# xiejihong0306/collision-detect-GJK-EPA

Measured on AMD Instinct MI355X. Metric: M convex-pair GJK+EPA queries/sec at 1/2/4/8 MI355X; % HBM roofline, higher is better.
Workload: dtype f64

## Files before the change

### collision-detect-gjk-epa_amd/csrc/gjkepa_kernel.h

```cpp
#pragma once
#include <hip/hip_runtime.h>

#include <cstddef>
#include <cstdint>

#ifndef GJKEPA_G0_G
#define GJKEPA_G0_G 4
#endif
#ifndef GJKEPA_G0_K
#define GJKEPA_G0_K 8
#endif
#ifndef GJKEPA_G0_MINW
#define GJKEPA_G0_MINW 2
#endif
#ifndef GJKEPA_G1_G
#define GJKEPA_G1_G 16
#endif
#ifndef GJKEPA_G1_K
#define GJKEPA_G1_K 8
#endif
#ifndef GJKEPA_G1_MINW
#define GJKEPA_G1_MINW 3
#endif
#ifndef GJKEPA_G2_G
// ... 50 lines not shown
#ifndef GJKEPA_E2_VCAP
#define GJKEPA_E2_VCAP 72
#endif
#ifndef GJKEPA_E2_FCAP
#define GJKEPA_E2_FCAP 128
#endif
#ifndef GJKEPA_E2_MINW
#define GJKEPA_E2_MINW 2
#endif
#ifndef GJKEPA_E2_REFILL
#define GJKEPA_E2_REFILL 1
#endif
#ifndef GJKEPA_E3_G
#define GJKEPA_E3_G 64
#endif
#ifndef GJKEPA_E3_K
#define GJKEPA_E3_K 4
#endif
#ifndef GJKEPA_E3_VCAP
#define GJKEPA_E3_VCAP 40
#endif
#ifndef GJKEPA_E3_FCAP
#define GJKEPA_E3_FCAP 64
#endif
#ifndef GJKEPA_E3_MINW
#define GJKEPA_E3_MINW 4
#endif
#ifndef GJKEPA_E4_G
#define GJKEPA_E4_G 64
#endif
#ifndef GJKEPA_E4_K
#define GJKEPA_E4_K 4
#endif
#ifndef GJKEPA_E4_VCAP
#define GJKEPA_E4_VCAP 104
#endif
#ifndef GJKEPA_E4_FCAP
#define GJKEPA_E4_FCAP 208
#endif
#ifndef GJKEPA_E4_MINW
#define GJKEPA_E4_MINW 2
#endif
#ifndef GJKEPA_E5_G
#define GJKEPA_E5_G 64
#endif
#ifndef GJKEPA_E5_K
#define GJKEPA_E5_K 4
#endif
#ifndef GJKEPA_E5_VCAP
#define GJKEPA_E5_VCAP 208
#endif
#ifndef GJKEPA_E5_FCAP
#define GJKEPA_E5_FCAP 416
#endif
#ifndef GJKEPA_E5_MINW
#define GJKEPA_E5_MINW 1
#endif
#ifndef GJKEPA_Q_VCAP
#define GJKEPA_Q_VCAP 40
#endif
#ifndef GJKEPA_Q_FCAP
#define GJKEPA_Q_FCAP 64
#endif
#ifndef GJKEPA_C0_G
#define GJKEPA_C0_G 8
#endif
#ifndef GJKEPA_C0_K
#define GJKEPA_C0_K 4
#endif
#ifndef GJKEPA_C0_MINW
#define GJKEPA_C0_MINW 3
#endif
#ifndef GJKEPA_C1_G
#define GJKEPA_C1_G 64
#endif
#ifndef GJKEPA_C1_K
#define GJKEPA_C1_K 4
#endif
#ifndef GJKEPA_C1_MINW
#define GJKEPA_C1_MINW 3
#endif
#ifndef GJKEPA_CT_QUEUE04
#define GJKEPA_CT_QUEUE04 1
#endif
#ifndef GJKEPA_SEED_HANDOFF
#define GJKEPA_SEED_HANDOFF 1
#endif
#ifndef GJKEPA_E1_PRIO
#define GJKEPA_E1_PRIO 2
#endif
#ifndef GJKEPA_SCREEN_MIN_K
#define GJKEPA_SCREEN_MIN_K 8
#endif
#ifndef GJKEPA_G0_LH
#define GJKEPA_G0_LH 1
#endif
#ifndef GJKEPA_G1_LH
#define GJKEPA_G1_LH 1
#endif
#ifndef GJKEPA_G2_LH
#define GJKEPA_G2_LH 1
#endif
#ifndef GJKEPA_E0_LH
#define GJKEPA_E0_LH 1
#endif
#ifndef GJKEPA_E1_LH
#define GJKEPA_E1_LH 0
#endif
#ifndef GJKEPA_E2_LH
#define GJKEPA_E2_LH 0
#endif
#ifndef GJKEPA_E3_LH
#define GJKEPA_E3_LH 1
#endif
#ifndef GJKEPA_E4_LH
#define GJKEPA_E4_LH 1
#endif
#ifndef GJKEPA_E5_LH
#define GJKEPA_E5_LH 0
#endif
#ifndef GJKEPA_C0_LH
#define GJKEPA_C0_LH 1
#endif
#ifndef GJKEPA_C1_LH
#define GJKEPA_C1_LH 1
#endif
#define GJKEPA_GJK_TIERS 3
#define GJKEPA_EPA_TIERS 6
#define GJKEPA_CONTACT_TIERS 2

#define GJKEPA_WS_COUNTERS 40
#define GJKEPA_WS_TALLY 48
#define GJKEPA_ROUTE_DONE 0
#define GJKEPA_ROUTE_GJK1 1
#define GJKEPA_ROUTE_EPA0 0x10
#define GJKEPA_ROUTE_CT0 0x20
#define GJKEPA_ROUTE_CT(t) (GJKEPA_ROUTE_CT0 + 2 * (t))
#define GJKEPA_ROUTE_REDO 0x2E
#define GJKEPA_TALLY_SEED_OWN 0x2D
#define GJKEPA_TALLY_SEED_HANDED 0x2F

#define GJKEPA_PARK_VC 72
#define GJKEPA_PARK_FC 128
#define GJKEPA_PARK_HDR 128
#define GJKEPA_PARK_BYTES (GJKEPA_PARK_HDR + 3 * 8 * GJKEPA_PARK_VC + 2 * 4 * GJKEPA_PARK_FC)

#define GJKEPA_GRID_UNITS (-2)

struct gjkepa_gjk_args {
    const void* verts;
    const int64_t* hull_off;
    const int32_t* hull_cnt;
    const int32_t* pairs;
    int64_t n_pairs;
    uint8_t* route;
    int route_code;
    uint32_t* ctr;
    int claim;
    uint32_t* tally;
    uint32_t* warm;
    void* out;
    int grid;
    int num_cus;
    uint32_t guard;
};

struct gjkepa_epa_args {
    int version;
    double tol_ff;
    const void* verts;
    const int64_t* hull_off;
    const int32_t* hull_cnt;
    const int32_t* pairs;
    int64_t n_pairs;
    uint8_t* route;
    int route_code;
    int next_code;
    int ct_base;
    uint32_t* ctr;
    int claim;
    uint32_t* tally;
    void* out;
    int grid;
    int num_cus;
    unsigned char* park;
    uint32_t* park_ctr;
    uint32_t park_cap;
    uint32_t guard;
};

__host__ __device__ inline uint64_t gjkepa_mix(uint64_t h, uint64_t v) {
    h ^= v + 0x9e3779b97f4a7c15ull + (h << 6) + (h >> 2);
    return h;
}
__host__ __device__ inline uint32_t gjkepa_fold(uint64_t h) { return (uint32_t)(h ^ (h >> 32)) | 1u; }
__host__ __device__ inline uint32_t gjkepa_guard_of(const gjkepa_gjk_args& a) {
    uint64_t h = 0x67ull;
    h = gjkepa_mix(h, (uint64_t)a.verts); h = gjkepa_mix(h, (uint64_t)a.hull_off); h = gjkepa_mix(h, (uint64_t)a.hull_cnt);
    h = gjkepa_mix(h, (uint64_t)a.pairs); h = gjkepa_mix(h, (uint64_t)a.n_pairs); h = gjkepa_mix(h, (uint64_t)a.route);
    h = gjkepa_mix(h, (uint64_t)(int64_t)a.route_code); h = gjkepa_mix(h, (uint64_t)a.ctr);
    h = gjkepa_mix(h, (uint64_t)(int64_t)a.claim); h = gjkepa_mix(h, (uint64_t)a.tally); h = gjkepa_mix(h, (uint64_t)a.warm);
    h = gjkepa_mix(h, (uint64_t)a.out); h = gjkepa_mix(h, (uint64_t)(int64_t)a.grid); h = gjkepa_mix(h, (uint64_t)(int64_t)a.num_cus);
    return gjkepa_fold(h);
}
__host__ __device__ inline uint32_t gjkepa_guard_of(const gjkepa_epa_args& a) {
    uint64_t h = 0x65ull;
    h = gjkepa_mix(h, (uint64_t)(int64_t)a.version); h = gjkepa_mix(h, __builtin_bit_cast(uint64_t, a.tol_ff));
    h = gjkepa_mix(h, (uint64_t)a.verts); h = gjkepa_mix(h, (uint64_t)a.hull_off); h = gjkepa_mix(h, (uint64_t)a.hull_cnt);
    h = gjkepa_mix(h, (uint64_t)a.pairs); h = gjkepa_mix(h, (uint64_t)a.n_pairs); h = gjkepa_mix(h, (uint64_t)a.route);
    h = gjkepa_mix(h, (uint64_t)(int64_t)a.route_code); h = gjkepa_mix(h, (uint64_t)(int64_t)a.next_code);
    h = gjkepa_mix(h, (uint64_t)(int64_t)a.ct_base); h = gjkepa_mix(h, (uint64_t)a.ctr);
    h = gjkepa_mix(h, (uint64_t)(int64_t)a.claim); h = gjkepa_mix(h, (uint64_t)a.tally); h = gjkepa_mix(h, (uint64_t)a.out);
    h = gjkepa_mix(h, (uint64_t)(int64_t)a.grid); h = gjkepa_mix(h, (uint64_t)(int64_t)a.num_cus);
    h = gjkepa_mix(h, (uint64_t)a.park); h = gjkepa_mix(h, (uint64_t)a.park_ctr); h = gjkepa_mix(h, (uint64_t)a.park_cap);
    return gjkepa_fold(h);
}

#ifndef GJKEPA_D0_MINW
#define GJKEPA_D0_MINW 2
#endif
#ifndef GJKEPA_D1_MINW
#define GJKEPA_D1_MINW 2
#endif
// ... 117 lines not shown
```

### collision-detect-gjk-epa_amd/csrc/gjkepa_kernel.hip

```cpp
#include <hip/hip_runtime.h>

#include <cfloat>
#include <cmath>
#include <cstdint>
#include <type_traits>

#include "../../include/gjkepa.h"
#include "gjkepa_kernel.h"
#include "gk_common.h"

#ifdef GK_PART
#define GK_IN(p) (GK_PART == (p))
#else
#define GK_IN(p) 1
#endif
#if GK_IN(12) || GK_IN(14)
#include "dist_simplex.h"
#endif
#if GK_IN(13)
#include "cast_advance.h"
#endif
#if GK_IN(14)
#include "manifold_clip.h"
#endif
// ... 1296 lines not shown
    const V3<T> q = vmk<T>(n.x, n.y, T(0));
    const T nq = norm2(q);
    nnew = vdiv(q, nq);
    return 0;
}

constexpr uint32_t kStale = 0xFFFFFFFFu;
constexpr int PH_MISS = 0, PH_HIT = -1;

CTX_T DEV V3<T> support_pt(const CTX& c, V3<T> d, uint32_t& code) {
    int ia, ib;
    support_idx(c, d, ia, ib);
    code = (uint32_t)ia | ((uint32_t)ib << 16);
    return vsub(c.A(ia), c.B(ib));
}
CTX_T DEV V3<T> decode_pt(const CTX& c, uint32_t code) {
    if (code == kStale) return zero3<T>();
    return vsub(c.A((int)(code & 0xffffu)), c.B((int)(code >> 16)));
}

CTX_T DEV void update_simplex_c(const CTX& c, V3<T> nq, V3<T>& s0, V3<T>& s1, V3<T>& s2, V3<T>& s3,
                                uint32_t& k0, uint32_t& k1, uint32_t& k2, uint32_t& k3) {
    const V3<T> M = centroid4(s0, s1, s2, s3), O = zero3<T>();
    const int q = c.g.gl & 3;
    const V3<T> ref = q == 3 ? s1 : s0;
    if (dot(nq, vsub(ref, M)) < T(0)) nq = vneg(nq);
    T best = dot(vneg(nq), vsub(ref, O));
    int k = q;
    V3<T> dir = nq;
#pragma unroll
    for (int st = 0; st < 2; ++st) {
        const T ob = st == 0 ? xchg<0>(best) : xchg<1>(best);
        const int ok = st == 0 ? xchg<0>(k) : xchg<1>(k);
        const V3<T> od = st == 0 ? vmk<T>(xchg<0>(dir.x), xchg<0>(dir.y), xchg<0>(dir.z))
                                 : vmk<T>(xchg<1>(dir.x), xchg<1>(dir.y), xchg<1>(dir.z));
        const bool take = ob > best || (ob == best && ok < k);
        best = take ? ob : best;
        k = take ? ok : k;
        dir = vsel(take, od, dir);
    }
    k = c.g.uni(k);
    uint32_t km;
    const V3<T> SM = support_pt(c, dir, km);
    const V3<T> o0 = s0, o1 = s1, o2 = s2;
    const uint32_t c0 = k0, c1 = k1, c2 = k2, c3 = k3;
    s0 = vsel(k == 3, o1, o0);
    s1 = vsel(k == 0 || k == 3, o2, o1);
    s2 = vsel(k == 2, o2, s3);
    s3 = SM;
    k0 = k == 3 ? c1 : c0;
    k1 = (k == 0 || k == 3) ? c2 : c1;
    k2 = k == 2 ? c2 : c3;
    k3 = km;
}

constexpr double kWarmMargin = 1e-6;
constexpr uint32_t kWarmMiss = 0xFFFFFFFEu;
CTX_T DEV bool warm_start(CTX& c, const uint32_t* w, uint32_t* kc) {
    uint32_t code[4];
    bool ok = true;
#pragma unroll
    for (int i = 0; i < 4; ++i) {
        code[i] = w[i];
        ok = ok && code[i] != kStale && (int)(code[i] & 0xffffu) < c.na && (int)(code[i] >> 16) < c.nb;
    }
    if (!c.g.unib(ok)) return false;
    const V3<T> s0 = decode_pt(c, code[0]), s1 = decode_pt(c, code[1]), s2 = decode_pt(c, code[2]), s3 = decode_pt(c, code[3]);
    const V3<T> M = centroid4(s0, s1, s2, s3), O = zero3<T>();
    const V3<T> P[4] = {s0, s1, s2, s3};
    const int F[4][3] = {{0, 2, 3}, {0, 1, 3}, {0, 1, 2}, {1, 2, 3}};
    bool inside = true;
#pragma unroll
    for (int f = 0; f < 4; ++f) {
        V3<T> n = face_nml(P[F[f][0]], P[F[f][1]], P[F[f][2]]);
        if (dot(n, vsub(P[F[f][0]], M)) < T(0)) n = vneg(n);
        inside = inside && dot(vsub(P[F[f][0]], O), n) > T(kWarmMargin);
    }
    if (!c.g.unib(inside)) return false;
#pragma unroll
    for (int i = 0; i < 4; ++i) kc[i] = code[i];
    return true;
}

CTX_T DEV int gjk_phase(CTX& c, uint32_t* kc, int& gjk_it, SeedOut<T>* so = nullptr) {
    const V3<T> O = zero3<T>();
    auto& L = c.L;
    const int gl = c.g.gl;
    gjk_it = 0;
    {
        T cs[(6 + G - 1) / G];
#pragma unroll
        for (int j0 = 0; j0 < 6; j0 += G) {
            const int j = j0 + gl;
            cs[j0 / G] = T(0);
            if (j < 6) {
                const int h = j / 3, ax = j - 3 * (j / 3);
                const TH* col = ax == 0 ? L.hx[h] : ax == 1 ? L.hy[h] : L.hz[h];
                const int n = h ? c.nb : c.na;
                T sum = 0;
                int i = 0;
                for (; i + 8 <= n; i += 8) {
                    TH v[8];
#pragma unroll
                    for (int u = 0; u < 8; ++u) v[u] = col[i + u];
#pragma unroll
                    for (int u = 0; u < 8; ++u) sum += (T)v[u];
                }
                for (; i < n; ++i) sum += (T)col[i];
                cs[j0 / G] = sum / (T)n;
            }
        }
        const int gb = c.g.lane & ~(G - 1);
        auto mc = [&](int j) { return __shfl(cs[j / G], gb + j % G); };
        const V3<T> m1 = vmk<T>(mc(0), mc(1), mc(2)), m2 = vmk<T>(mc(3), mc(4), mc(5));
        T r1 = -Tol<T>::BIG, r2 = -Tol<T>::BIG;
#pragma unroll
        for (int k = 0; k < K; ++k) {
            int i = k * G + gl;
            const V3<T> da = vsub(c.AV(k), m1);
            const T ta = da.x * da.x + da.y * da.y + da.z * da.z;
            if (i < c.na && ta > r1) r1 = ta;
            const V3<T> db = vsub(c.BV(k), m2);
            const T tb = db.x * db.x + db.y * db.y + db.z * db.z;
            if (i < c.nb && tb > r2) r2 = tb;
        }
        r1 = tsqrt(gmax<G>(r1));
        r2 = tsqrt(gmax<G>(r2));
        GK_STAMP(SG_SPHERE);
        if (!c.g.unib(norm2(vsub(m1, m2)) <= r1 + r2 + T(1))) return PH_MISS;
    }
    V3<T> s0 = O, s1 = O, s2 = O, s3 = O;
    uint32_t k0 = kStale, k1 = kStale, k2 = kStale, k3 = kStale;
    V3<T> dir;
    for (int iter = 1;; ++iter) {
        if (iter > 99) return PH_MISS;
        dir = vmk<T>((T)kDirTab[iter - 1][0], (T)kDirTab[iter - 1][1], (T)kDirTab[iter - 1][2]);
        s0 = support_pt(c, dir, k0);
        dir = vneg(dir);
        s1 = support_pt(c, dir, k1);
        if (!c.g.unib(allclose8(s0, s1))) break;
    }
    dir = vec_pl(O, s0, s1);
    s2 = support_pt(c, dir, k2);
    if (c.g.unib(allclose8(s2, s0) || allclose8(s2, s1))) return PH_MISS;
    dir = utzvec(cross(vsub(s1, s0), vsub(s2, s1)));
    const T vd = dot(vsub(O, s2), dir);
    bool enter = false;
    if (c.g.unib(fabs(vd) < Tol<T>::PT) && c.g.unib(inside_tri(s0, s1, s2, O))) enter = true;
    const bool tri = enter;
    const int q = gl & 3;
    V3<T> nq = zero3<T>();
    T mdq = 0;
    if (!enter) {
        if (c.g.unib(vd < T(0))) dir = vneg(dir);
        s3 = support_pt(c, dir, k3);
        const V3<T> n = uninml(s0, s1, s2);
        if (c.g.unib(is_zero_nml(n))) return GJKEPA_STATUS_DEGENERATE;
        if (c.g.unib(fabs(dot(vsub(s3, s0), n)) < Tol<T>::PT)) return PH_MISS;
        nq = quad_normal(q, s0, s1, s2, s3, mdq);
        if (c.g.unib(quad_inside(q, s0, s1, s2, s3, nq))) enter = true;
    }
    GK_STAMP(SG_INIT);
    if (!enter) {
        constexpr int HS = (12 + G - 1) / G;
        T h1[HS], h2[HS];
#pragma unroll
        for (int t = 0; t < HS; ++t) { h1[t] = 0; h2[t] = 0; }
        const uint64_t lowg = G == 64 ? ~0ull : ((1ull << (G & 63)) - 1ull);
        const int sh = c.g.lane & ~(G - 1);
        for (int it = 1;; ++it) {
            gjk_it = it;
            if (it > 50) return PH_MISS;
#pragma unroll
            for (int t = 0; t < HS; ++t) {
                const int j = t * G + gl;
                h2[t] = h1[t];
                h1[t] = simplex_coord(j < 12 ? j : 0, s0, s1, s2, s3);
            }
            GK_STAMP(SG_CHK);
            update_simplex_c(c, nq, s0, s1, s2, s3, k0, k1, k2, k3);
            nq = quad_normal(q, s0, s1, s2, s3, mdq);
            GK_STAMP(SG_UPD);
            if (c.g.unib(qbcast<2>(mdq) < Tol<T>::PT)) return PH_MISS;
            const V3<T> n = vmk<T>(qbcast<2>(nq.x), qbcast<2>(nq.y), qbcast<2>(nq.z));
            if (c.g.unib(fabs(dot(vsub(s3, s0), n)) < Tol<T>::PT)) return PH_MISS;
            if (c.g.unib(quad_inside(q, s0, s1, s2, s3, nq))) break;
            uint32_t e1 = 0, e2 = 0;
#pragma unroll
            for (int t = 0; t < HS; ++t) {
                const int j = t * G + gl;
                const T cur = simplex_coord(j < 12 ? j : 0, s0, s1, s2, s3);
                e1 |= (uint32_t)((__ballot(fabs(cur - h1[t]) < Tol<T>::PT) >> sh) & lowg) << (t * G);
                e2 |= (uint32_t)((__ballot(fabs(cur - h2[t]) < Tol<T>::PT) >> sh) & lowg) << (t * G);
            }
            e1 &= 0xFFFu;
            e2 &= 0xFFFu;
            bool over = true;
#pragma unroll
            for (int p = 0; p < 4; ++p) over = over && (((e1 >> (3 * p)) & 7u) == 7u || ((e2 >> (3 * p)) & 7u) == 7u);
            if (c.g.unib(over)) return PH_MISS;
        }
        GK_STAMP(SG_CHK);
    }
    kc[0] = k0; kc[1] = k1; kc[2] = k2; kc[3] = k3;
    if constexpr (handoff<T>()) {
        if (so) {
            const bool same_bits = c.g.unib(quad_all(mdq > T(4) * Tol<T>::Z && nq.x != T(0) && nq.y != T(0) && nq.z != T(0)));
            so->nq = nq;
            so->ok = !tri && same_bits && simplex_is_first_tetra(c.g, s0, s1, s2, s3);
        }
    }
    return PH_HIT;
}

CTX_T DEV int epa_phase(CTX& c, const uint32_t* kc, T& depth, V3<T>& n, uint32_t& diag_epa, bool park = false,
                        ParkCtl pk = {}, const unsigned char* rec = nullptr, uint32_t* gjk_it = nullptr,
                        SeedIn<T> h = no_seed<T>()) {
    V3<T> s0 = zero3<T>(), s1 = s0, s2 = s0, s3 = s0;
    if (!rec) { s0 = decode_pt(c, kc[0]); s1 = decode_pt(c, kc[1]); s2 = decode_pt(c, kc[2]); s3 = decode_pt(c, kc[3]); }
    depth = 0;
    n = zero3<T>();
    int eit = 0, nf = 0;
    const int st = epa(c, s0, s1, s2, s3, depth, n, eit, nf, park, pk, rec, gjk_it, h);
    diag_epa = ((uint32_t)(eit & 0xff) << 8) | ((uint32_t)(nf & 0xffff) << 16);
    return st;
}

template <bool DEFER = false, typename T, typename TH, int G, int K, int VC, int FC, int LH>
DEV int contact_phase(CTX& c, T depth, V3<T> n, int version, T tol_ff, T* o13, Pend04* pd = nullptr) {
    int st;
    int ia, ib;
    GK_STAMP(SE_TERM);
    DotSet<T, K> D;
    support_dots(c, n, D, ia, ib);
    GK_STAMP(SE_NEAR);
    V3<T> pt = zero3<T>();
    int type = (version == 1 || version == 2) ? collision_type(c, D, tol_ff) : 0;
    if (version == 1) st = contact_v1(c, n, D, pt);
    else if (version == 2) st = contact_v2<DEFER>(c, D, pt, pd);
    else if (version == 3) { V3<T> nw; st = contact_v3(c, n, pt, nw); n = nw; }
    else st = GJKEPA_STATUS_BAD_VERSION;
    GK_STAMP(SE_CONT);
    if (st) return st;
    if (version == 3) type = collision_type(c, n, tol_ff);
    GK_STAMP(SE_TYPE);
    const V3<T> q1 = c.A(ia), q2 = c.B(ib);
    __builtin_amdgcn_wave_barrier();
    o13[0] = depth;
    o13[1] = n.x; o13[2] = n.y; o13[3] = n.z;
    o13[4] = pt.x; o13[5] = pt.y; o13[6] = pt.z;
    o13[7] = q1.x; o13[8] = q1.y; o13[9] = q1.z;
    o13[10] = q2.x; o13[11] = q2.y; o13[12] = q2.z;
    return -type;
}

CTX_T DEV bool load_hulls(CTX& c, const TH* __restrict__ pa, const TH* __restrict__ pb) {
    const int gl = c.g.gl;
    bool nonfinite = false;
    constexpr bool kScreen = (ScreenOn<K>::value && sizeof(T) == 8 && sizeof(TH) == 4) || certify<T>();
    float ma = 0.0f, mb = 0.0f;
#pragma unroll
    for (int k = 0; k < K; ++k) {
        const int i = k * G + gl;
        TH ax = 0, ay = 0, az = 0, bx = 0, by = 0, bz = 0;
        const int ja = i < c.na ? i : 0, jb = i < c.nb ? i : 0;
        if (i < c.na || c.na > 0) { ax = pa[ja]; ay = pa[c.na + ja]; az = pa[2 * c.na + ja]; }
        if (i < c.nb || c.nb > 0) { bx = pb[jb]; by = pb[c.nb + jb]; bz = pb[2 * c.nb + jb]; }
        nonfinite = nonfinite || !isfinite(ax) || !isfinite(ay) || !isfinite(az) || !isfinite(bx) ||
                    !isfinite(by) || !isfinite(bz);
        if constexpr (kScreen) {
            ma = fmaxf(ma, fmaxf(fabsf((float)ax), fmaxf(fabsf((float)ay), fabsf((float)az))));
            mb = fmaxf(mb, fmaxf(fabsf((float)bx), fmaxf(fabsf((float)by), fabsf((float)bz))));
        }
        if constexpr (CTX::kRegHull) {
            c.ax[k] = (T)ax; c.ay[k] = (T)ay; c.az[k] = (T)az;
            c.bx[k] = (T)bx; c.by[k] = (T)by; c.bz[k] = (T)bz;
        }
        c.L.hx[0][i] = ax; c.L.hy[0][i] = ay; c.L.hz[0][i] = az;
        c.L.hx[1][i] = bx; c.L.hy[1][i] = by; c.L.hz[1][i] = bz;
    }
    if constexpr (kScreen) {
        c.vmax_a = gmax<G>(ma);
        c.vmax_b = gmax<G>(mb);
// ... 111 lines not shown
}
DEV void tally_route(uint8_t code) { if (code < GJKEPA_WS_TALLY) atomicAdd(&s_tally[code], 1u); }
DEV void tally_end(uint32_t* tally) {
    __builtin_amdgcn_fence(__ATOMIC_SEQ_CST, "workgroup");
    __builtin_amdgcn_wave_barrier();
    const int l = lane_id();
    if (l < GJKEPA_WS_TALLY && s_tally[l]) atomicAdd(&tally[l], s_tally[l]);
}
DEV bool tier_empty(const uint32_t* tally, int route_code) {
    return route_code >= 0 && __builtin_amdgcn_readfirstlane(tally[route_code]) == 0;
}
DEV int pick_claim(const uint32_t* tally, int route_code, int64_t n_pairs, int claim) {
    if (route_code < 0 || claim <= 1) return claim;
    const uint32_t mine = __builtin_amdgcn_readfirstlane(tally[route_code]);
    return (int64_t)mine * 16 >= n_pairs ? 1 : claim;
}

template <int G, bool META = false, typename F, typename R = NoRoundHook>
DEV void for_each_routed_pair(const Grp<G>& grp, int64_t n_pairs, const uint8_t* __restrict__ route, int route_code,
                              uint32_t* ctr, int claim, bool unit_grid, F&& f, const int32_t* pairs = nullptr,
                              const int32_t* cnt = nullptr, const int64_t* off = nullptr, R&& after = R{}) {
    const int64_t nchunks = (n_pairs + 63) / 64;
    uint32_t next = 0;
    if (unit_grid) {
        const int64_t u = blockIdx.x;
        if (u < nchunks) {
            const int64_t p0 = u * 64;
            const int len = n_pairs - p0 < 64 ? (int)(n_pairs - p0) : 64;
            const uint64_t m = route_code < 0 ? (len >= 64 ? ~0ull : ((1ull << len) - 1ull))
                                              : __ballot(grp.lane < len && (int)route[p0 + grp.lane] == route_code);
            groups_take<G, META>(grp, p0, m, pairs, cnt, off, f, after);
        }
        return;
    }
    if (claim <= 1 || route_code < 0) {
        const Units U(n_pairs, tail_unit<G, (64 / G > 8 ? 64 / G : 8)>(n_pairs));
        if ((int64_t)blockIdx.x < U.nunits && grp.lane == 0) next = gridDim.x + atomicAdd(ctr, 1u);
        int64_t u = blockIdx.x;
        while (u < U.nunits) {
            if (grp.lane == 0 && u != (int64_t)blockIdx.x) next = gridDim.x + atomicAdd(ctr, 1u);
            int64_t p0;
            int len;
            U.range(u, p0, len);
            uint64_t m;
            if (route_code < 0) {
                m = len >= 64 ? ~0ull : ((1ull << len) - 1ull);
            } else {
                const int64_t p = p0 + grp.lane;
                m = __ballot(grp.lane < len && (int)route[p] == route_code);
            }
            groups_take<G, META>(grp, p0, m, pairs, cnt, off, f, after);
            u = (int64_t)__builtin_amdgcn_readfirstlane(next);
        }
        return;
    }
    const int64_t nunits = (nchunks + 15) / 16;
    if ((int64_t)blockIdx.x < nunits && grp.lane == 0) next = gridDim.x + atomicAdd(ctr, 1u);
    for (int64_t run = blockIdx.x; run * 16 < nchunks; run = (int64_t)__builtin_amdgcn_readfirstlane(next)) {
        if (grp.lane == 0 && run != (int64_t)blockIdx.x) next = gridDim.x + atomicAdd(ctr, 1u);
        const int64_t q0 = run * 1024 + 16 * grp.lane;
        uint4 v = make_uint4(0xFFFFFFFFu, 0xFFFFFFFFu, 0xFFFFFFFFu, 0xFFFFFFFFu);
        if (q0 + 16 <= n_pairs) {
            v = *reinterpret_cast<const uint4*>(route + q0);
        } else {
            uint32_t w[4] = {0xFFFFFFFFu, 0xFFFFFFFFu, 0xFFFFFFFFu, 0xFFFFFFFFu};
            for (int i = 0; i < 16; ++i)
                if (q0 + i < n_pairs) w[i >> 2] = (w[i >> 2] & ~(0xffu << (8 * (i & 3)))) | ((uint32_t)route[q0 + i] << (8 * (i & 3)));
            v = make_uint4(w[0], w[1], w[2], w[3]);
        }
        const uint32_t mine = match16(v, (uint32_t)route_code);
        uint64_t lanes = __ballot(mine != 0);
        while (lanes) {
            const int j = (int)__builtin_ctzll(lanes) >> 2;
            lanes &= ~(0xFull << (4 * j));
            uint64_t m = 0;
#pragma unroll
            for (int i = 0; i < 4; ++i)
                m |= (uint64_t)(uint32_t)__builtin_amdgcn_readlane((int)mine, 4 * j + i) << (16 * i);
            groups_take<G, META>(grp, run * 1024 + 64 * j, m, pairs, cnt, off, f, after);
        }
    }
}

template <typename TIn, typename T, int G, int K, int MINW, bool LH, bool WARM>
__global__ __launch_bounds__(64, MINW) void gjk_kernel(const gjkepa_gjk_args a) {
    static_assert(G >= 4, "the tetrahedron faces run on quads");
    using L_t = Lds<T, TIn, G, K, 0, 0>;
    extern __shared__ __align__(16) unsigned char smem[];
    const Grp<G> grp;
    L_t& L = *reinterpret_cast<L_t*>(smem + lds_stride<L_t, G>() * (grp.lane / G));
    const int gl = grp.gl;
    const TIn* verts = (const TIn*)a.verts;
    GK_GUARD(1, a.route_code);
    GK_STAMP_BEGIN();
    if (tier_empty(a.tally, a.route_code)) return;
    tally_begin();
    const int claim = pick_claim(a.tally, a.route_code, a.n_pairs, a.claim);
    auto body = [&](int64_t pair, const PairMeta& pm) {
        GK_STAMP(SG_ROUTE);
        Ctx<T, TIn, G, K, 0, 0, LH> c{L, grp};
        const int na = grp.uni(pm.na), nb = grp.uni(pm.nb);
        T o13[13];
#pragma unroll
        for (int i = 0; i < 13; ++i) o13[i] = T(0);
        uint8_t next = 0;
        if (na < 1 || nb < 1 || na > GJKEPA_MAX_HULL_VERTS || nb > GJKEPA_MAX_HULL_VERTS) {
            store_record<G, T>(a.out, pair, gl, o13, 0, 0, GJKEPA_STATUS_BAD_INPUT, 0u);
            if (WARM && gl < 4) a.warm[4 * pair + gl] = kStale;
        } else if (na > K * G || nb > K * G) {
            next = (uint8_t)((na > nb ? na : nb) <= GJKEPA_G1_G * GJKEPA_G1_K ? GJKEPA_ROUTE_GJK1 : GJKEPA_ROUTE_GJK1 + 1);
        } else {
            c.na = na;
            c.nb = nb;
            const bool bad_in = load_hulls(c, verts + pm.oa, verts + pm.ob);
            GK_STAMP(SG_LOAD);
            if (bad_in) {
                store_record<G, T>(a.out, pair, gl, o13, 0, 0, GJKEPA_STATUS_BAD_INPUT, 0u);
                if (WARM && gl < 4) a.warm[4 * pair + gl] = kStale;
            } else {
                uint32_t kc[4];
                int gjk_it = 0;
                int r = PH_MISS;
                bool warm_hit = false;
                if constexpr (WARM) {
                    if (a.warm[4 * pair] != kWarmMiss) warm_hit = warm_start(c, a.warm + 4 * pair, kc);
                }
                SeedOut<T> so{zero3<T>(), false};
                if (warm_hit) r = PH_HIT;
                else r = gjk_phase(c, kc, gjk_it, &so);
                __builtin_amdgcn_wave_barrier();
                GK_STAMP(SG_CHK);
                if (WARM && gl < 4)
                    a.warm[4 * pair + gl] = r == PH_HIT ? (gl == 0 ? kc[0] : gl == 1 ? kc[1] : gl == 2 ? kc[2] : kc[3])
                                          : (r == PH_MISS && gl == 0) ? kWarmMiss : kStale;
                if (r == PH_HIT) {
#pragma unroll
                    for (int j0 = 0; j0 < 6; j0 += G) {
                        const int j = j0 + gl;
                        const uint32_t word = j == 0 ? kc[0] : j == 1 ? kc[1] : j == 2 ? kc[2] : j == 3 ? kc[3] : j == 4 ? (uint32_t)gjk_it : 0u;
                        if (j < 6) reinterpret_cast<uint32_t*>(a.out)[pair * (sizeof(T) == 8 ? 32 : 16) + j] = word;
                    }
                    if constexpr (handoff<T>()) {
                        uint32_t* slot = reinterpret_cast<uint32_t*>(a.out) + pair * 32;
                        if (so.ok && gl < 4) {
                            const int f = gl == 0 ? 1 : gl == 1 ? 2 : gl == 2 ? 0 : 3;
                            T* np = reinterpret_cast<T*>(slot + kSeedNmlWord) + 3 * f;
                            np[0] = so.nq.x; np[1] = so.nq.y; np[2] = so.nq.z;
                        }
                        if (gl == 0) slot[kSeedFlagWord] = so.ok ? 1u : 0u;
                    }
                    next = (uint8_t)(GJKEPA_ROUTE_EPA0 + epa_tier_for(na > nb ? na : nb));
                } else if (r == PH_MISS) {
                    store_record<G, T>(a.out, pair, gl, o13, 0, 0, 0, 0u);
                } else if (certify<T>()) {
                    next = GJKEPA_ROUTE_REDO;
                } else {
                    store_record<G, T>(a.out, pair, gl, o13, 1, 0, r, (uint32_t)(gjk_it & 0xff));
                }
            }
        }
        if (gl == 0) { a.route[pair] = next; tally_route(next); }
        __builtin_amdgcn_wave_barrier();
        GK_STAMP(SG_STORE);
    };
    for_each_routed_pair<G, true>(grp, a.n_pairs, a.route, a.route_code, a.ctr, claim, false, body, a.pairs, a.hull_cnt,
                                  a.hull_off);
    GK_STAMP(SG_ROUTE);
    tally_end(a.tally);
    GK_STAMP_END();
}

DEV int contact_tier_for(int nmax) { return nmax <= GJKEPA_C0_G * GJKEPA_C0_K ? 0 : 1; }

template <typename TIn, typename T, int G, int K, int VC, int FC, int MINW, bool LH, int PR>
__global__ __launch_bounds__(64, MINW) void epa_kernel(const gjkepa_epa_args a) {
    using L_t = Lds<T, TIn, G, K, VC, FC>;
    extern __shared__ __align__(16) unsigned char smem[];
    const Grp<G> grp;
    L_t& L = *reinterpret_cast<L_t*>(smem + lds_stride<L_t, G>() * (grp.lane / G));
    const int gl = grp.gl;
    const TIn* verts = (const TIn*)a.verts;
    GK_GUARD(2, a.route_code);
    GK_STAMP_BEGIN();
    if (tier_empty(a.tally, a.route_code)) return;
    tally_begin();
    const int claim = pick_claim(a.tally, a.route_code, a.n_pairs, a.claim);
    for_each_routed_pair<G>(grp, a.n_pairs, a.route, a.route_code, a.ctr, claim, false, [&](int64_t pair) {
        GK_STAMP(SE_ROUTE);
        Ctx<T, TIn, G, K, VC, FC, LH> c{L, grp};
        const int32_t ha = a.pairs[2 * pair], hb = a.pairs[2 * pair + 1];
        c.na = grp.uni(a.hull_cnt[ha]);
        c.nb = grp.uni(a.hull_cnt[hb]);
        uint32_t* slot = reinterpret_cast<uint32_t*>(a.out) + pair * (sizeof(T) == 8 ? 32 : 16);
        uint32_t kc[4];
        kc[0] = slot[0]; kc[1] = slot[1]; kc[2] = slot[2]; kc[3] = slot[3];
        const uint32_t gjk_it = slot[4];
        load_hulls(c, verts + a.hull_off[ha], verts + a.hull_off[hb]);
        T depth;
        V3<T> n;
        uint32_t de = 0;
        GK_STAMP(SE_LOAD);
#ifdef GJKEPA_DIAG_GJK_ONLY
        const int r = GJKEPA_STATUS_DEGENERATE;
        depth = 0; n = zero3<T>();
#else
        const uint32_t parked = (PR & 2) && a.park ? slot[5] : 0u;
        uint32_t it_park = gjk_it;
        const ParkCtl pk{a.park, a.park_ctr, a.park_cap, gjk_it, slot};
        const bool can_park = (PR & 1) && a.park && a.next_code >= 0;
        const bool fits = c.na <= G * K && c.nb <= G * K;
        const SeedIn<T> seed = load_seed<T>(slot, gl);
        if (fits && !parked && gl == 0) tally_route(seed.on ? GJKEPA_TALLY_SEED_HANDED : GJKEPA_TALLY_SEED_OWN);
        const int r = !fits ? ST_DEFER
                    : epa_phase(c, kc, depth, n, de, can_park, pk,
                                parked ? a.park + (size_t)(parked - 1) * GJKEPA_PARK_BYTES : nullptr, &it_park, seed);
#endif
        __builtin_amdgcn_wave_barrier();
        const uint32_t diag = (gjk_it & 0xffu) | de;
        uint8_t next = 0;
        if ((r == ST_DEFER || r == ST_PARKED) && a.next_code >= 0) {
            next = (uint8_t)(GJKEPA_ROUTE_EPA0 + epa_tier_for(c.na > c.nb ? c.na : c.nb, a.next_code - GJKEPA_ROUTE_EPA0, VC));
        } else if (redo_status<T>(r, a.next_code < 0)) {
            next = GJKEPA_ROUTE_REDO;
        } else if (r == 0) {
            T* rec = reinterpret_cast<T*>(slot);
            if (gl < 4) rec[gl] = gl == 0 ? depth : gl == 1 ? n.x : gl == 2 ? n.y : n.z;
            if (gl == 4) slot[sizeof(T) == 8 ? 27 : 14] = diag;
            next = (uint8_t)(a.ct_base + contact_tier_for(c.na > c.nb ? c.na : c.nb));
        } else {
            T o13[13];
#pragma unroll
            for (int i = 0; i < 13; ++i) o13[i] = T(0);
            store_record<G, T>(a.out, pair, gl, o13, 1, 0, r == ST_DEFER ? GJKEPA_STATUS_DEGENERATE : r, diag);
        }
        if (gl == 0) { a.route[pair] = next; tally_route(next); }
        __builtin_amdgcn_wave_barrier();
        GK_STAMP(SE_STORE);
    });
    GK_STAMP(SE_ROUTE);
    tally_end(a.tally);
    GK_STAMP_END();
}

struct PairQueue {
    const uint8_t* route;
    Units U;
    int64_t ch, p0;
// ... 781 lines not shown
        c.nb = grp.uni(pm.nb);
        if (load_hulls(c, verts + pm.oa, verts + pm.ob)) {
            if (gl == 0) store_manifold_empty(a.out, pair, GJKEPA_STATUS_BAD_INPUT, 0);
            __builtin_amdgcn_wave_barrier();
            return;
        }
        V3<T> n;
        manifold_hit(a.records, pair, a.rec_stride, a.rec_hit_off, n);
        const unsigned char* rec = a.records + pair * (int64_t)a.rec_stride;
        gkm::D3 cp;
        if (a.rec_stride == (int)sizeof(gjkepa_contact_f64)) {
            const double* d = reinterpret_cast<const double*>(rec);
            cp = gkm::mk(d[4], d[5], d[6]);
        } else {
            const float* d = reinterpret_cast<const float*>(rec);
            cp = gkm::mk((double)d[4], (double)d[5], (double)d[6]);
        }
        T ta[K], tb[K];
        T va = -Tol<T>::BIG, vb = Tol<T>::BIG;
#pragma unroll
        for (int k = 0; k < K; ++k) {
            const V3<T> p = c.AV(k), q = c.BV(k);
            ta[k] = n.x * p.x + n.y * p.y + n.z * p.z;
            tb[k] = n.x * q.x + n.y * q.y + n.z * q.z;
            va = red_max(ta[k], va);
            vb = red_min(tb[k], vb);
        }
        const T hA = gmax<G>(va) + T(0), hB = gmin<G>(vb) + T(0);
        const int fa = manifold_feature<G, K>(grp, ta, c.na, hA - a.margin, false, L.feat[0]);
        const int fb = manifold_feature<G, K>(grp, tb, c.nb, hB + a.margin, true, L.feat[1]);
        __builtin_amdgcn_wave_barrier();
        MfMem<C, L_t> mem{c, L};
        const gkm::Patch p = gkm::clip_manifold(mem, gkm::mk(n.x, n.y, n.z), hA, gkm::decimated_count(fa),
                                                gkm::decimated_count(fb), cp);
        const int flags = p.flags | ((fa > gkm::kMaxFeature || fb > gkm::kMaxFeature) ? GJKEPA_MANIFOLD_DECIMATED : 0);
        uint64_t w[20];
        w[0] = __builtin_bit_cast(uint64_t, hA - hB);
        w[1] = __builtin_bit_cast(uint64_t, n.x);
        w[2] = __builtin_bit_cast(uint64_t, n.y);
        w[3] = __builtin_bit_cast(uint64_t, n.z);
#pragma unroll
        for (int k = 0; k < 4; ++k) {
            w[4 + 3 * k] = __builtin_bit_cast(uint64_t, p.pt[k].x);
            w[5 + 3 * k] = __builtin_bit_cast(uint64_t, p.pt[k].y);
            w[6 + 3 * k] = __builtin_bit_cast(uint64_t, p.pt[k].z);
        }
        w[16] = (uint64_t)p.code[0] | ((uint64_t)p.code[1] << 32);
        w[17] = (uint64_t)p.code[2] | ((uint64_t)p.code[3] << 32);
        w[18] = (uint64_t)(uint32_t)(fa & 0xffff) | ((uint64_t)(uint32_t)(fb & 0xffff) << 16) |
                ((uint64_t)((uint32_t)(p.n & 0xff) | ((uint32_t)GJKEPA_STATUS_OK << 8) | ((uint32_t)(flags & 0xff) << 16)) << 32);
        w[19] = __builtin_bit_cast(uint64_t, p.area);
        __builtin_amdgcn_wave_barrier();
        store_manifold<G>(a.out, pair, gl, w);
        __builtin_amdgcn_wave_barrier();
    };
    for_each_dist_pair<G, G * K, TIER, true>(grp, a, body);
}
#endif

}

hipError_t gk_launch_query_f32(int vert_dtype, const gjkepa_epa_args& a, hipStream_t s);
#define GK_EPA_DECL(t) hipError_t gk_launch_epa_##t(int vert_dtype, int precision, const gjkepa_epa_args& a, hipStream_t s);
GK_EPA_DECL(0) GK_EPA_DECL(1) GK_EPA_DECL(2) GK_EPA_DECL(3) GK_EPA_DECL(4) GK_EPA_DECL(5)
static_assert(GJKEPA_EPA_TIERS == 6, "one launcher per EPA tier");
namespace {

template <int G> int grid_cap(int64_t n_pairs, int grid) {
    const int64_t chunks = (n_pairs + 63) / 64, rounds = (n_pairs + 64 / G - 1) / (64 / G);
    const int64_t want = rounds <= (int64_t)grid * 8 / (64 / G) ? rounds : chunks;
    return (int)(want < 1 ? 1 : want < grid ? want : grid);
}
template <typename K_t> int grid_for(K_t kfn, size_t lds, int num_cus, int grid) {
    if (grid > 0) return grid;
    int per_cu = 0;
    if (hipOccupancyMaxActiveBlocksPerMultiprocessor(&per_cu, kfn, 64, lds) != hipSuccess || per_cu < 1) per_cu = 1;
    return per_cu * num_cus;
}

#if GK_IN(2)
template <typename TIn, typename T, int G, int K, int MINW, bool LH>
hipError_t launch_gjk(const gjkepa_gjk_args& a, hipStream_t s) {
    auto kfn = a.warm ? gk::gjk_kernel<TIn, T, G, K, MINW, LH, true> : gk::gjk_kernel<TIn, T, G, K, MINW, LH, false>;
    constexpr int GPW = 64 / G;
    const size_t lds = gk::lds_stride<gk::Lds<T, TIn, G, K, 0, 0>, G>() * GPW;
    int grid = grid_for(kfn, lds, a.num_cus, a.grid);
    grid = grid_cap<G>(a.n_pairs, grid);
    hipLaunchKernelGGL(kfn, dim3(grid), dim3(64), lds, s, a);
    return hipGetLastError();
}
template <typename TIn, typename T>
hipError_t gjk_any(int tier, const gjkepa_gjk_args& a, hipStream_t s) {
    static_assert(GJKEPA_GJK_TIERS == 3 && GJKEPA_G2_G * GJKEPA_G2_K >= GJKEPA_MAX_HULL_VERTS, "the last GJK tier holds every hull");
    return tier == 0 ? launch_gjk<TIn, T, GJKEPA_G0_G, GJKEPA_G0_K, GJKEPA_G0_MINW, (GJKEPA_G0_LH != 0)>(a, s)
         : tier == 1 ? launch_gjk<TIn, T, GJKEPA_G1_G, GJKEPA_G1_K, GJKEPA_G1_MINW, (GJKEPA_G1_LH != 0)>(a, s)
                     : launch_gjk<TIn, T, GJKEPA_G2_G, GJKEPA_G2_K, GJKEPA_G2_MINW, (GJKEPA_G2_LH != 0)>(a, s);
}
#endif

template <typename TIn, typename T, int G, int K, int VC, int FC, int MINW, bool LH, int REFILL = 0, int PR = 0>
hipError_t launch_epa(const gjkepa_epa_args& a, hipStream_t s) {
    auto kfn = [] {
        if constexpr (REFILL > 0) return gk::epa_kernel_refill<TIn, T, G, K, VC, FC, MINW, LH, REFILL, PR>;
        else return gk::epa_kernel<TIn, T, G, K, VC, FC, MINW, LH, PR>;
    }();
    constexpr int GPW = 64 / G;
    const size_t lds = gk::lds_stride<gk::Lds<T, TIn, G, K, VC, FC>, G>() * GPW;
    int grid = grid_for(kfn, lds, a.num_cus, a.grid);
    grid = grid_cap<G>(a.n_pairs, grid);
    hipLaunchKernelGGL(kfn, dim3(grid), dim3(64), lds, s, a);
    return hipGetLastError();
}

#define EPA_ARGS(t) GJKEPA_E##t##_G, GJKEPA_E##t##_K, GJKEPA_E##t##_VCAP, GJKEPA_E##t##_FCAP, GJKEPA_E##t##_MINW, \
                    (GJKEPA_E##t##_LH != 0)

#if GK_IN(3)
template <typename TIn, typename T, int G, int K, int MINW, bool LH>
hipError_t launch_contact(const gjkepa_epa_args& a, hipStream_t s) {
    auto kfn = gk::contact_kernel<TIn, T, G, K, MINW, LH>;
    const size_t lds = gk::contact_lds_bytes<TIn, T, G, K>();
    int grid;
    if (a.grid == GJKEPA_GRID_UNITS) {
        grid = (int)((a.n_pairs + 63) / 64);
    } else {
        grid = grid_cap<G>(a.n_pairs, grid_for(kfn, lds, a.num_cus, a.grid));
    }
    hipLaunchKernelGGL(kfn, dim3(grid), dim3(64), lds, s, a);
    return hipGetLastError();
}
template <typename TIn, typename T>
hipError_t contact_any(int tier, const gjkepa_epa_args& a, hipStream_t s) {
    if (tier == 0)
        return launch_contact<TIn, T, GJKEPA_C0_G, GJKEPA_C0_K, GJKEPA_C0_MINW, (GJKEPA_C0_LH != 0)>(a, s);
    return launch_contact<TIn, T, GJKEPA_C1_G, GJKEPA_C1_K, GJKEPA_C1_MINW, (GJKEPA_C1_LH != 0)>(a, s);
}
#endif

#define GK_EPA_DEF(t, ...)                                                                                        \
    hipError_t gk_launch_epa_##t(int vert_dtype, int precision, const gjkepa_epa_args& a, hipStream_t s) {          \
        if (vert_dtype == GJKEPA_DTYPE_F32)                                                                         \
            return precision == GJKEPA_PREC_F64 ? launch_epa<float, double, __VA_ARGS__>(a, s)                      \
                                                : launch_epa<float, float, __VA_ARGS__>(a, s);                      \
        return precision == GJKEPA_PREC_F64 ? launch_epa<double, double, __VA_ARGS__>(a, s)                        \
                                            : launch_epa<double, float, __VA_ARGS__>(a, s);                         \
    }

}

#if GK_IN(4)
GK_EPA_DEF(0, EPA_ARGS(0), GJKEPA_E0_REFILL)
#endif
#if GK_IN(5)
GK_EPA_DEF(1, EPA_ARGS(1), GJKEPA_E1_REFILL)
#endif
#if GK_IN(6)
GK_EPA_DEF(2, EPA_ARGS(2), GJKEPA_E2_REFILL, 1)
#endif
#if GK_IN(7)
GK_EPA_DEF(3, EPA_ARGS(3), 0, 1)
#endif
#if GK_IN(8)
GK_EPA_DEF(4, EPA_ARGS(4), 0, 2)
#endif
#if GK_IN(9)
GK_EPA_DEF(5, EPA_ARGS(5))
#endif

// ... 158 lines not shown
```

Measured before the change: 197.1.

## Defer long-running GJK pairs into an LDS queue and resume them in batches

In the small-group GJK tier, a pair stops iterating once too few lane groups in the wave are still active. Its simplex codes and history go into an LDS ring, and stopped pairs are resumed later in full-wave batches. The aim is to cut divergence waste, where a few slow pairs hold a whole wave. The cost is extra LDS per block, which can lower occupancy, plus hull reloads and simplex re-decoding on resume. The path is only enabled for 4-byte input vertices with groups of 4 lanes or fewer.

```diff
diff --git a/collision-detect-gjk-epa_amd/csrc/gjkepa_kernel.h b/collision-detect-gjk-epa_amd/csrc/gjkepa_kernel.h
--- a/collision-detect-gjk-epa_amd/csrc/gjkepa_kernel.h
+++ b/collision-detect-gjk-epa_amd/csrc/gjkepa_kernel.h
@@ -156,6 +156,12 @@
 #endif
 #ifndef GJKEPA_CT_QUEUE04
 #define GJKEPA_CT_QUEUE04 1
+#endif
+#ifndef GJKEPA_G0_DEFER_AT
+#define GJKEPA_G0_DEFER_AT 7
+#endif
+#ifndef GJKEPA_G0_REPUSH
+#define GJKEPA_G0_REPUSH 0
 #endif
 #ifndef GJKEPA_SEED_HANDOFF
 #define GJKEPA_SEED_HANDOFF 1
@@ -213,6 +219,7 @@
 #define GJKEPA_ROUTE_REDO 0x2E
 #define GJKEPA_TALLY_SEED_OWN 0x2D
 #define GJKEPA_TALLY_SEED_HANDED 0x2F
+#define GJKEPA_TALLY_GJK_QUEUED 0x2C
 
 #define GJKEPA_PARK_VC 72
 #define GJKEPA_PARK_FC 128
diff --git a/collision-detect-gjk-epa_amd/csrc/gjkepa_kernel.hip b/collision-detect-gjk-epa_amd/csrc/gjkepa_kernel.hip
--- a/collision-detect-gjk-epa_amd/csrc/gjkepa_kernel.hip
+++ b/collision-detect-gjk-epa_amd/csrc/gjkepa_kernel.hip
@@ -1402,12 +1402,32 @@
     return true;
 }
 
-CTX_T DEV int gjk_phase(CTX& c, uint32_t* kc, int& gjk_it, SeedOut<T>* so = nullptr) {
+constexpr int PH_STOP = -3;
+constexpr int GJK_STOPS = 1;
+constexpr int GJK_RESUMES = 2;
+struct GjkStop {
+    uint32_t k[4];
+    uint64_t hk1, hk2;
+    int it;
+};
+DEV uint64_t codes_pack(uint32_t k0, uint32_t k1, uint32_t k2, uint32_t k3) {
+    auto h = [](uint32_t k) { return (k & 0xffu) | ((k >> 8) & 0xff00u); };
+    return (uint64_t)(h(k0) | (h(k1) << 16)) | ((uint64_t)(h(k2) | (h(k3) << 16)) << 32);
+}
+DEV uint32_t codes_at(uint64_t p, int i) {
+    const uint32_t h = (uint32_t)(p >> (16 * i)) & 0xffffu;
+    return h == 0xffffu ? kStale : (h & 0xffu) | ((h >> 8) << 16);
+}
+
+template <int MODE = 0, typename T, typename TH, int G, int K, int VC, int FC, int LH>
+DEV int gjk_phase(CTX& c, uint32_t* kc, int& gjk_it, SeedOut<T>* so = nullptr, [[maybe_unused]] GjkStop* st = nullptr,
+              [[maybe_unused]] int defer_at = 0) {
+    constexpr bool FRESH = (MODE & GJK_RESUMES) == 0;
     const V3<T> O = zero3<T>();
     auto& L = c.L;
     const int gl = c.g.gl;
     gjk_it = 0;
-    {
+    if constexpr (FRESH) {
         T cs[(6 + G - 1) / G];
 #pragma unroll
         for (int j0 = 0; j0 < 6; j0 += G) {
@@ -1452,7 +1472,7 @@
     V3<T> s0 = O, s1 = O, s2 = O, s3 = O;
     uint32_t k0 = kStale, k1 = kStale, k2 = kStale, k3 = kStale;
     V3<T> dir;
-    for (int iter = 1;; ++iter) {
+    for (int iter = 1; FRESH; ++iter) {
         if (iter > 99) return PH_MISS;
         dir = vmk<T>((T)kDirTab[iter - 1][0], (T)kDirTab[iter - 1][1], (T)kDirTab[iter - 1][2]);
         s0 = support_pt(c, dir, k0);
@@ -1460,18 +1480,25 @@
         s1 = support_pt(c, dir, k1);
         if (!c.g.unib(allclose8(s0, s1))) break;
     }
-    dir = vec_pl(O, s0, s1);
-    s2 = support_pt(c, dir, k2);
-    if (c.g.unib(allclose8(s2, s0) || allclose8(s2, s1))) return PH_MISS;
-    dir = utzvec(cross(vsub(s1, s0), vsub(s2, s1)));
-    const T vd = dot(vsub(O, s2), dir);
+    if constexpr (FRESH) {
+        dir = vec_pl(O, s0, s1);
+        s2 = support_pt(c, dir, k2);
+        if (c.g.unib(allclose8(s2, s0) || allclose8(s2, s1))) return PH_MISS;
+        dir = utzvec(cross(vsub(s1, s0), vsub(s2, s1)));
+    }
+    const T vd = FRESH ? dot(vsub(O, s2), dir) : T(0);
     bool enter = false;
-    if (c.g.unib(fabs(vd) < Tol<T>::PT) && c.g.unib(inside_tri(s0, s1, s2, O))) enter = true;
+    if (FRESH && c.g.unib(fabs(vd) < Tol<T>::PT) && c.g.unib(inside_tri(s0, s1, s2, O))) enter = true;
     const bool tri = enter;
     const int q = gl & 3;
     V3<T> nq = zero3<T>();
     T mdq = 0;
-    if (!enter) {
+    if constexpr (!FRESH) {
+        k0 = st->k[0]; k1 = st->k[1]; k2 = st->k[2]; k3 = st->k[3];
+        s0 = decode_pt(c, k0); s1 = decode_pt(c, k1); s2 = decode_pt(c, k2); s3 = decode_pt(c, k3);
+        nq = quad_normal(q, s0, s1, s2, s3, mdq);
+    }
+    if (FRESH && !enter) {
         if (c.g.unib(vd < T(0))) dir = vneg(dir);
         s3 = support_pt(c, dir, k3);
         const V3<T> n = uninml(s0, s1, s2);
@@ -1486,9 +1513,23 @@
         T h1[HS], h2[HS];
 #pragma unroll
         for (int t = 0; t < HS; ++t) { h1[t] = 0; h2[t] = 0; }
+        [[maybe_unused]] uint64_t hk1 = ~0ull, hk2 = ~0ull;
+        if constexpr (!FRESH) {
+            hk1 = st->hk1; hk2 = st->hk2;
+            const V3<T> a0 = decode_pt(c, codes_at(hk1, 0)), a1 = decode_pt(c, codes_at(hk1, 1)),
+                        a2 = decode_pt(c, codes_at(hk1, 2)), a3 = decode_pt(c, codes_at(hk1, 3));
+            const V3<T> b0 = decode_pt(c, codes_at(hk2, 0)), b1 = decode_pt(c, codes_at(hk2, 1)),
+                        b2 = decode_pt(c, codes_at(hk2, 2)), b3 = decode_pt(c, codes_at(hk2, 3));
+#pragma unroll
+            for (int t = 0; t < HS; ++t) {
+                const int j = t * G + gl;
+                h1[t] = simplex_coord(j < 12 ? j : 0, a0, a1, a2, a3);
+                h2[t] = simplex_coord(j < 12 ? j : 0, b0, b1, b2, b3);
+            }
+        }
         const uint64_t lowg = G == 64 ? ~0ull : ((1ull << (G & 63)) - 1ull);
         const int sh = c.g.lane & ~(G - 1);
-        for (int it = 1;; ++it) {
+        for (int it = FRESH ? 1 : st->it + 1;; ++it) {
             gjk_it = it;
             if (it > 50) return PH_MISS;
 #pragma unroll
@@ -1496,6 +1537,11 @@
                 const int j = t * G + gl;
                 h2[t] = h1[t];
                 h1[t] = simplex_coord(j < 12 ? j : 0, s0, s1, s2, s3);
+            }
+            if constexpr ((MODE & GJK_STOPS) != 0) {
+                static_assert(G * K < 255, "codes_pack keeps a vertex index in a byte");
+                hk2 = hk1;
+                hk1 = codes_pack(k0, k1, k2, k3);
             }
             GK_STAMP(SG_CHK);
             update_simplex_c(c, nq, s0, s1, s2, s3, k0, k1, k2, k3);
@@ -1519,6 +1565,14 @@
 #pragma unroll
             for (int p = 0; p < 4; ++p) over = over && (((e1 >> (3 * p)) & 7u) == 7u || ((e2 >> (3 * p)) & 7u) == 7u);
             if (c.g.unib(over)) return PH_MISS;
+            if constexpr ((MODE & GJK_STOPS) != 0) {
+                if (popc(__ballot(true)) <= defer_at * G) {
+                    st->k[0] = k0; st->k[1] = k1; st->k[2] = k2; st->k[3] = k3;
+                    st->hk1 = hk1; st->hk2 = hk2;
+                    st->it = it;
+                    return PH_STOP;
+                }
+            }
         }
         GK_STAMP(SG_CHK);
     }
@@ -1796,6 +1850,120 @@
     }
 }
 
+template <bool WARM, int G, typename T>
+DEV uint8_t gjk_finish(void* out, uint32_t* warm, int64_t pair, int gl, int na, int nb, int r, const uint32_t* kc,
+                       int gjk_it, const SeedOut<T>& so, const T* o13) {
+    uint8_t next = 0;
+    if (WARM && gl < 4)
+        warm[4 * pair + gl] = r == PH_HIT ? (gl == 0 ? kc[0] : gl == 1 ? kc[1] : gl == 2 ? kc[2] : kc[3])
+                            : (r == PH_MISS && gl == 0) ? kWarmMiss : kStale;
+    if (r == PH_HIT) {
+#pragma unroll
+        for (int j0 = 0; j0 < 6; j0 += G) {
+            const int j = j0 + gl;
+            const uint32_t word = j == 0 ? kc[0] : j == 1 ? kc[1] : j == 2 ? kc[2] : j == 3 ? kc[3] : j == 4 ? (uint32_t)gjk_it : 0u;
+            if (j < 6) reinterpret_cast<uint32_t*>(out)[pair * (sizeof(T) == 8 ? 32 : 16) + j] = word;
+        }
+        if constexpr (handoff<T>()) {
+            uint32_t* slot = reinterpret_cast<uint32_t*>(out) + pair * 32;
+            if (so.ok && gl < 4) {
+                const int f = gl == 0 ? 1 : gl == 1 ? 2 : gl == 2 ? 0 : 3;
+                T* np = reinterpret_cast<T*>(slot + kSeedNmlWord) + 3 * f;
+                np[0] = so.nq.x; np[1] = so.nq.y; np[2] = so.nq.z;
+            }
+            if (gl == 0) slot[kSeedFlagWord] = so.ok ? 1u : 0u;
+        }
+        next = (uint8_t)(GJKEPA_ROUTE_EPA0 + epa_tier_for(na > nb ? na : nb));
+    } else if (r == PH_MISS) {
+        store_record<G, T>(out, pair, gl, o13, 0, 0, 0, 0u);
+    } else if (certify<T>()) {
+        next = GJKEPA_ROUTE_REDO;
+    } else {
+        store_record<G, T>(out, pair, gl, o13, 1, 0, r, (uint32_t)(gjk_it & 0xff));
+    }
+    return next;
+}
+
+struct PendGjkEntry {
+    int64_t pair, oa, ob;
+    uint64_t hk1, hk2;
+    uint32_t k[4];
+    int32_t na, nb, it, pad;
+};
+template <int G> struct PendGjkQueue {
+    static constexpr int CAP = 2 * (64 / G);
+    PendGjkEntry e[CAP];
+};
+template <int G, typename TIn> constexpr bool gjk_queue() { return GJKEPA_G0_DEFER_AT > 0 && 64 / G >= 16 && sizeof(TIn) == 4; }
+template <typename TIn, typename T, int G, int K> constexpr size_t gjk_lds_bytes() {
+    size_t bytes = lds_stride<Lds<T, TIn, G, K, 0, 0>, G>() * (64 / G);
+    if constexpr (gjk_queue<G, TIn>()) bytes += sizeof(PendGjkQueue<G>);
+    return bytes;
+}
+template <int G>
+DEV int gjk_queue_push(PendGjkQueue<G>& Q, int qhead, int qn, const Grp<G>& grp, bool stopped, int64_t pair, int64_t oa,
+                       int64_t ob, int na, int nb, const GjkStop& st) {
+    const uint64_t pushing = __ballot(stopped);
+    if (stopped && grp.gl == 0) {
+        const int rank = popc(pushing & ((1ull << grp.lane) - 1ull)) / G;
+        auto& e = Q.e[(qhead + qn + rank) & (PendGjkQueue<G>::CAP - 1)];
+        e.pair = pair; e.oa = oa; e.ob = ob;
+        e.hk1 = st.hk1; e.hk2 = st.hk2;
+        e.k[0] = st.k[0]; e.k[1] = st.k[1]; e.k[2] = st.k[2]; e.k[3] = st.k[3];
+        e.na = na; e.nb = nb; e.it = st.it; e.pad = 0;
+    }
+    __builtin_amdgcn_wave_barrier();
+    return popc(pushing) / G;
+}
+
+template <typename TIn, typename T, int G, int K, bool LH, bool WARM>
+DEV int gjk_queue_round(int qhead, int cnt, int qn, int defer_at, const TIn* verts, void* out, uint8_t* route,
+                        uint32_t* warm) {
+    using L_t = Lds<T, TIn, G, K, 0, 0>;
+    using Q_t = PendGjkQueue<G>;
+    extern __shared__ __align__(16) unsigned char smem[];
+    const Grp<G> grp;
+    const int gl = grp.gl, g = grp.lane / G;
+    L_t& L = *reinterpret_cast<L_t*>(smem + lds_stride<L_t, G>() * g);
+    Q_t& Q = *reinterpret_cast<Q_t*>(smem + lds_stride<L_t, G>() * (64 / G));
+    int64_t pair = 0, oa = 0, ob = 0;
+    int na = 0, nb = 0;
+    GjkStop st{{kStale, kStale, kStale, kStale}, ~0ull, ~0ull, 0};
+    if (g < cnt) {
+        const auto& e = Q.e[(qhead + g) & (Q_t::CAP - 1)];
+        pair = e.pair; oa = e.oa; ob = e.ob;
+        st.hk1 = e.hk1; st.hk2 = e.hk2;
+        st.k[0] = e.k[0]; st.k[1] = e.k[1]; st.k[2] = e.k[2]; st.k[3] = e.k[3];
+        na = e.na; nb = e.nb; st.it = e.it;
+    }
+    __builtin_amdgcn_wave_barrier();
+    bool stopped = false;
+    if (g < cnt) {
+        Ctx<T, TIn, G, K, 0, 0, LH> c{L, grp};
+        c.na = na;
+        c.nb = nb;
+        load_hulls(c, verts + oa, verts + ob);
+        GK_STAMP(SG_LOAD);
+        uint32_t kc[4];
+        int gjk_it = 0;
+        SeedOut<T> so{zero3<T>(), false};
+        const int r = gjk_phase<GJK_RESUMES | (GJKEPA_G0_REPUSH != 0 ? GJK_STOPS : 0)>(c, kc, gjk_it, &so, &st, defer_at);
+        stopped = r == PH_STOP;
+        if (!stopped) {
+            __builtin_amdgcn_wave_barrier();
+            T o13[13];
+#pragma unroll
+            for (int i = 0; i < 13; ++i) o13[i] = T(0);
+            const uint8_t next = gjk_finish<WARM, G, T>(out, warm, pair, gl, na, nb, r, kc, gjk_it, so, o13);
+            if (gl == 0) { route[pair] = next; tally_route(next); tally_route(GJKEPA_TALLY_GJK_QUEUED); }
+        }
+    }
+    int pushed = 0;
+    if constexpr (GJKEPA_G0_REPUSH != 0) pushed = gjk_queue_push<G>(Q, qhead, qn, grp, stopped, pair, oa, ob, na, nb, st);
+    __builtin_amdgcn_wave_barrier();
+    return pushed;
+}
+
 template <typename TIn, typename T, int G, int K, int MINW, bool LH, bool WARM>
 __global__ __launch_bounds__(64, MINW) void gjk_kernel(const gjkepa_gjk_args a) {
     static_assert(G >= 4, "the tetrahedron faces run on quads");
@@ -1810,6 +1978,12 @@
     if (tier_empty(a.tally, a.route_code)) return;
     tally_begin();
     const int claim = pick_claim(a.tally, a.route_code, a.n_pairs, a.claim);
+    constexpr bool QG = gjk_queue<G, TIn>();
+    constexpr int GPW = 64 / G;
+    using Q_t = PendGjkQueue<G>;
+    static_assert(lds_stride<L_t, G>() % 8 == 0, "the ring follows the images, 8-byte aligned");
+    [[maybe_unused]] int qhead = 0, qn = 0;
+    [[maybe_unused]] bool pushed = false;
     auto body = [&](int64_t pair, const PairMeta& pm) {
         GK_STAMP(SG_ROUTE);
         Ctx<T, TIn, G, K, 0, 0, LH> c{L, grp};
@@ -1840,43 +2014,46 @@
                     if (a.warm[4 * pair] != kWarmMiss) warm_hit = warm_start(c, a.warm + 4 * pair, kc);
                 }
                 SeedOut<T> so{zero3<T>(), false};
+                [[maybe_unused]] GjkStop st;
                 if (warm_hit) r = PH_HIT;
+                else if constexpr (QG) r = gjk_phase<GJK_STOPS>(c, kc, gjk_it, &so, &st, GJKEPA_G0_DEFER_AT);
                 else r = gjk_phase(c, kc, gjk_it, &so);
                 __builtin_amdgcn_wave_barrier();
                 GK_STAMP(SG_CHK);
-                if (WARM && gl < 4)
-                    a.warm[4 * pair + gl] = r == PH_HIT ? (gl == 0 ? kc[0] : gl == 1 ? kc[1] : gl == 2 ? kc[2] : kc[3])
-                                          : (r == PH_MISS && gl == 0) ? kWarmMiss : kStale;
-                if (r == PH_HIT) {
-#pragma unroll
-                    for (int j0 = 0; j0 < 6; j0 += G) {
-                        const int j = j0 + gl;
-                        const uint32_t word = j == 0 ? kc[0] : j == 1 ? kc[1] : j == 2 ? kc[2] : j == 3 ? kc[3] : j == 4 ? (uint32_t)gjk_it : 0u;
-                        if (j < 6) reinterpret_cast<uint32_t*>(a.out)[pair * (sizeof(T) == 8 ? 32 : 16) + j] = word;
+                if constexpr (QG) {
+                    if (r == PH_STOP) {
+                        Q_t& Q = *reinterpret_cast<Q_t*>(smem + lds_stride<L_t, G>() * GPW);
+                        gjk_queue_push<G>(Q, qhead, qn, grp, true, pair, pm.oa, pm.ob, na, nb, st);
+                        pushed = true;
+                        GK_STAMP(SG_STORE);
+                        return;
                     }
-                    if constexpr (handoff<T>()) {
-                        uint32_t* slot = reinterpret_cast<uint32_t*>(a.out) + pair * 32;
-                        if (so.ok && gl < 4) {
-                            const int f = gl == 0 ? 1 : gl == 1 ? 2 : gl == 2 ? 0 : 3;
-                            T* np = reinterpret_cast<T*>(slot + kSeedNmlWord) + 3 * f;
-                            np[0] = so.nq.x; np[1] = so.nq.y; np[2] = so.nq.z;
-                        }
-                        if (gl == 0) slot[kSeedFlagWord] = so.ok ? 1u : 0u;
-                    }
-                    next = (uint8_t)(GJKEPA_ROUTE_EPA0 + epa_tier_for(na > nb ? na : nb));
-                } else if (r == PH_MISS) {
-                    store_record<G, T>(a.out, pair, gl, o13, 0, 0, 0, 0u);
-                } else if (certify<T>()) {
-                    next = GJKEPA_ROUTE_REDO;
-                } else {
-                    store_record<G, T>(a.out, pair, gl, o13, 1, 0, r, (uint32_t)(gjk_it & 0xff));
                 }
+                next = gjk_finish<WARM, G, T>(a.out, a.warm, pair, gl, na, nb, r, kc, gjk_it, so, o13);
             }
         }
         if (gl == 0) { a.route[pair] = next; tally_route(next); }
         __builtin_amdgcn_wave_barrier();
         GK_STAMP(SG_STORE);
     };
+    if constexpr (QG) {
+        auto rounds = [&](int defer_at) __attribute__((always_inline)) {
+            const int cnt = qn < GPW ? qn : GPW;
+            const int back = gjk_queue_round<TIn, T, G, K, LH, WARM>(qhead, cnt, qn, defer_at, verts, a.out, a.route, a.warm);
+            qhead = (qhead + cnt) & (Q_t::CAP - 1);
+            qn += __builtin_amdgcn_readfirstlane(back) - cnt;
+            GK_STAMP(SG_STORE);
+        };
+        auto after = [&]() __attribute__((always_inline)) {
+            qn += popc(__ballot(pushed)) / G;
+            pushed = false;
+            while (qn >= GPW) rounds(GJKEPA_G0_REPUSH != 0 ? GJKEPA_G0_DEFER_AT : 0);
+        };
+        for_each_routed_pair<G, true>(grp, a.n_pairs, a.route, a.route_code, a.ctr, claim, false, body, a.pairs, a.hull_cnt,
+                                      a.hull_off, after);
+        GK_STAMP(SG_ROUTE);
+        while (qn > 0) rounds(0);
+    } else
     for_each_routed_pair<G, true>(grp, a.n_pairs, a.route, a.route_code, a.ctr, claim, false, body, a.pairs, a.hull_cnt,
                                   a.hull_off);
     GK_STAMP(SG_ROUTE);
@@ -2824,8 +3001,7 @@
 template <typename TIn, typename T, int G, int K, int MINW, bool LH>
 hipError_t launch_gjk(const gjkepa_gjk_args& a, hipStream_t s) {
     auto kfn = a.warm ? gk::gjk_kernel<TIn, T, G, K, MINW, LH, true> : gk::gjk_kernel<TIn, T, G, K, MINW, LH, false>;
-    constexpr int GPW = 64 / G;
-    const size_t lds = gk::lds_stride<gk::Lds<T, TIn, G, K, 0, 0>, G>() * GPW;
+    const size_t lds = gk::gjk_lds_bytes<TIn, T, G, K>();
     int grid = grid_for(kfn, lds, a.num_cus, a.grid);
     grid = grid_cap<G>(a.n_pairs, grid);
     hipLaunchKernelGGL(kfn, dim3(grid), dim3(64), lds, s, a);
```

Measured after the change: 202.2, median of 6. +2.6%, better.
